# BaratiLab/GAMD

Measured on AMD Instinct MI355X. Metric: atom-steps/sec (force eval + integrate), 10k-atom LJ box, higher is better.
Workload: dtype f32; 1 GPU; C2: 10 000-atom LJ box, rho*=0.5, L=92.29 A, cutoff 3.0 sigma=10.2 A, fp32, 4 conv layers x 128, random-init weights (seed 0), 1 box per GPU; n_atoms=10000, boxes=1, launch=single process

## Files before the change

gamd_amd/_lib.py:

```python
from __future__ import annotations

import ctypes as C
import os

_HERE = os.path.dirname(os.path.abspath(__file__))
LIB_PATH = os.environ.get("GAMD_LIB") or os.path.join(_HERE, "libgamd_hip.so")


class GamdConfig(C.Structure):
    _fields_ = [("n_atoms", C.c_int32), ("kind", C.c_int32), ("n_layers", C.c_int32),
                ("use_bond", C.c_int32), ("nbr_flavour", C.c_int32), ("device", C.c_int32),
                ("cutoff", C.c_float), ("box", C.c_float * 3), ("edge_capacity", C.c_int64),
                ("keep_stages", C.c_int32), ("edge_dtype", C.c_int32),
                ("encoding_size", C.c_int32), ("edge_embedding_dim", C.c_int32), ("hidden_dim", C.c_int32),
                ("no_expand_edge", C.c_int32), ("neighbor_skin", C.c_float), ("self_loop_mode", C.c_int32),
                ("kernel_select", C.c_int32), ("small_tile_limit", C.c_int32), ("n_boxes", C.c_int32)]


_MD_EXT = [("mass_h_amu", C.c_float), ("length_per_nm", C.c_float), ("rigid_water", C.c_int32),
           ("r_oh", C.c_float), ("r_hh", C.c_float), ("remove_cm_motion", C.c_int32)]


class GamdNhcParams(C.Structure):
    _fields_ = [("dt_ps", C.c_float), ("mass_amu", C.c_float), ("temperature_k", C.c_float),
# ... 45 lines not shown
TRAJ_FIELDS = {"x": 1, "v": 2, "f": 4, "image": 8}
FORCE_SOURCE = {"network": 0, "classical": 1}


_vp, _i32, _i64 = C.c_void_p, C.c_int32, C.c_int64
SYMBOLS = {
    "gamd_version": (C.c_char_p, []),
    "gamd_last_error": (C.c_char_p, []),
    "gamd_create": (_i32, [C.POINTER(GamdConfig), C.POINTER(_vp)]),
    "gamd_destroy": (_i32, [_vp]),
    "gamd_load_weight": (_i32, [_vp, C.c_char_p, _vp, C.POINTER(_i64), _i32]),
    "gamd_finalize_weights": (_i32, [_vp]),
    "gamd_set_scaler": (_i32, [_vp, C.c_double, C.c_double]),
    "gamd_set_bonds": (_i32, [_vp, _vp, _i64]),
    "gamd_forces_async": (_i32, [_vp, _vp, _vp, C.POINTER(C.c_float), _vp, _vp, _vp]),
    "gamd_set_node_features": (_i32, [_vp, _vp]),
    "gamd_get_device_flags": (_i32, [_vp, C.POINTER(_i32)]),
    "gamd_sync_status": (_i32, [_vp, _vp]),
    "gamd_forces_host": (_i32, [_vp, _vp, _vp, C.POINTER(C.c_float), _vp, _i32, _vp]),
    "gamd_forces": (_i32, [_vp, _vp, _vp, C.POINTER(C.c_float), _vp, _vp, _vp]),
    "gamd_forces_edges": (_i32, [_vp, _vp, _vp, C.POINTER(C.c_float), _vp, _vp, _i64, _vp, _vp, _vp]),
    "gamd_build_neighbors": (_i32, [_vp, _vp, _vp, C.POINTER(C.c_float), _vp]),
    "gamd_get_counts": (_i32, [_vp, C.POINTER(_i64), C.POINTER(_i64), C.POINTER(_i64)]),
    "gamd_get_skin_stats": (_i32, [_vp, C.POINTER(_i64), C.POINTER(_i64), C.POINTER(_i64)]),
    "gamd_debug_get": (_i32, [_vp, _i32, _vp, C.c_size_t]),
    "gamd_md_run": (_i32, [_vp, _vp, _vp, _vp, _vp, C.POINTER(C.c_float), C.POINTER(GamdMdParams), _i64, _vp]),
    "gamd_md_run_nhc": (_i32, [_vp, _vp, _vp, _vp, _vp, C.POINTER(C.c_float), C.POINTER(GamdNhcParams), _vp, _i64, _vp]),
    "gamd_report_configure": (_i32, [_vp, C.POINTER(GamdReportParams)]),
    "gamd_report_reset": (_i32, [_vp]),
    "gamd_report_read": (_i32, [_vp, _vp, _vp, _vp, _vp, _i64, C.POINTER(_i64), _vp, _i64, C.POINTER(_i64), C.POINTER(_i64),
                                C.POINTER(_i32)]),
    "gamd_traj_configure": (_i32, [_vp, C.POINTER(GamdTrajParams)]),
    "gamd_traj_reset": (_i32, [_vp]),
    "gamd_traj_read_frames": (_i32, [_vp, _vp, _i64, _i64, _vp, _vp, _vp, _vp, _vp, C.POINTER(_i64), C.POINTER(_i64)]),
    "gamd_traj_read_dynamics": (_i32, [_vp, _vp, _vp, _vp, _i64, C.POINTER(_i64), C.POINTER(C.c_uint64), _vp, C.POINTER(_i32)]),
    "gamd_struct_configure": (_i32, [_vp, C.POINTER(GamdStructParams)]),
    "gamd_struct_reset": (_i32, [_vp]),
    "gamd_struct_read": (_i32, [_vp, _vp, _vp, _i64, _vp, _i64, _vp, _i64, C.POINTER(_i64), C.POINTER(_i32)]),
    "gamd_classical_configure": (_i32, [_vp, C.POINTER(GamdClassicalParams)]),
    "gamd_classical_reset": (_i32, [_vp]),
    "gamd_classical_read": (_i32, [_vp, _vp, _vp, _vp, _i64, C.POINTER(_i64), C.POINTER(_i64), _vp, _i64]),
    "gamd_classical_eval": (_i32, [_vp, _vp, C.POINTER(C.c_float), C.c_float, _vp, _vp, _vp, _vp, _vp]),
    "gamd_md_force_source": (_i32, [_vp, _i32]),
    "gamd_minimize": (_i32, [_vp, _vp, C.POINTER(C.c_float), C.c_float, _vp, _vp, C.POINTER(GamdMinimizeParams), _vp, _vp]),
    "gamd_water_configure": (_i32, [_vp, C.POINTER(GamdWaterParams)]),
    "gamd_water_reset": (_i32, [_vp]),
# ... 41 lines not shown
```

gamd_amd/csrc/conv_edge.hip:

```cpp
#include "gamd_common.h"
#include "gamd_internal.h"

#include <cstdlib>

namespace {

constexpr int conv_lds_floats(bool l0) { return 2 * GAMD_WFRAG_FLOATS + 3 * 128; }

template <bool F2, typename Post, typename Mid>
__device__ __forceinline__ void gemm128_post(const f32x4* W, int lane, const f32x16 (&X)[4], f32x16 (&acc)[4], Post post, Mid mid) {
#pragma unroll
    for (int tp = 0; tp < 4; ++tp) {
        if (tp == 1) mid();
#pragma unroll
        for (int t = 0; t < 4; ++t) {
#pragma unroll
            for (int q = 0; q < 4; ++q) {
                const f32x4 w = W[((tp * 4 + t) * 4 + q) * 64 + lane];
#pragma unroll
                for (int j = 0; j < 4; ++j) {
                    const float x = X[t][q * 4 + j];
                    acc[tp] = F2 ? mfma32(x, w[j], acc[tp]) : mfma32(w[j], x, acc[tp]);
                }
                if (tp > 0) post(tp - 1, t * 4 + q);
            }
        }
    }
#pragma unroll
    for (int g = 0; g < 16; ++g) post(3, g);
}

template <int N>
__device__ __forceinline__ void phase_barrier() {
    asm volatile("s_waitcnt vmcnt(%0) lgkmcnt(0)" ::"n"(N) : "memory");
    __builtin_amdgcn_s_barrier();
}

__device__ __forceinline__ void load_e_tile(const float* __restrict__ e_frag, int tile, int lane, f32x16 (&X)[4]) {
    const f32x4* ef = (const f32x4*)e_frag + (size_t)tile * 16 * 64;
#pragma unroll
    for (int t = 0; t < 4; ++t)
#pragma unroll
        for (int q = 0; q < 4; ++q) {
            const f32x4 v = gamd_load_stream(&ef[(t * 4 + q) * 64 + lane]);
#pragma unroll
            for (int j = 0; j < 4; ++j) X[t][q * 4 + j] = v[j];
        }
}

template <bool TIME, bool L0>
__global__ void __launch_bounds__(512, 2) k_conv_edge(ConvEdgeArgs a) {
    if (a.devflags[DEVFLAG_FROZEN]) return;
    extern __shared__ __attribute__((aligned(16))) float lds[];
    float* buf0 = lds + (L0 ? 3 * 128 : 0);
    float* buf1 = buf0 + GAMD_WFRAG_FLOATS;
    float* vb1 = L0 ? lds : buf1 + GAMD_WFRAG_FLOATS;
    float* vb3 = vb1 + 128;
    float* vb4 = vb3 + 128;
    float* vSD0 = vb4;

    const int tid = threadIdx.x, lane = tid & 63, slot = lane & 31, half = lane >> 5;
    const int wave = __builtin_amdgcn_readfirstlane(tid >> 6);
    const unsigned lane16 = (unsigned)lane * 16u;
    int E = a.counters[CNT_E];
    if ((long long)E > a.e_cap) E = (int)a.e_cap;
    const int n_tiles = (E + GAMD_TILE - 1) / GAMD_TILE;
    const int n_units = (n_tiles + 3) / 4;
    int first, end, step;
    gamd_xcd_range(n_units, blockIdx.x, gridDim.x, first, end, step);
    if (first >= end) return;
    const int n_iter = ((end - first + step - 1) / step + 1) / 2;
    const int wsub = wave & 3, whalf = wave >> 2;
    const bool early = whalf == 0;
    auto tile_of = [&](int it) {
        const int u = first + (2 * it + whalf) * step;
        return (it < n_iter && u < end) ? u * 4 + wsub : n_tiles;
    };
    auto stage = [&](const float* gw, float* buf) { gamd_stage_weight_raw_contig<8>(gw, buf, wave, lane16); };

    long long tacc[16];
#pragma unroll
    for (int i = 0; i < 16; ++i) tacc[i] = 0;
    long long tprev = 0;
#define TMARK(i) do { if (TIME) { const long long tn__ = (long long)__builtin_readcyclecounter(); tacc[i] += tn__ - tprev; tprev = tn__; } } while (0)

    if (tid < 128) {
        vb1[tid] = a.b1[tid]; vb3[tid] = a.b3[tid];
        if (L0) vSD0[tid] = a.S[tid] + a.D[tid];
        else vb4[tid] = a.b4[tid];
    }
    stage(a.w1p, buf0);

    f32x16 RA[4], RB[4], RC[4];
    auto init_b4 = [&]() {
// ... 105 lines not shown
            gemm128_post<false>((const f32x4*)by, lane, RB, RA,
                                [&](int tp, int g) { RA[tp][g] = gamd_silu_hw(RA[tp][g]); },
                                [&]() { FENCE(); stage(a.w3p, bx); FENCE(); });
            TMARK(4);
        } else {
            stage(a.w3p, bx);
        }
        phase_barrier<0>();
        asm volatile("" ::"v"(mask), "v"(p0), "v"(src_n));
        TMARK(5);
        if (active) {
            const unsigned bl = (unsigned)__ballot(src != a.zero_row) >> (4 * half);
            const unsigned real = (bl & 0xFu) | ((bl >> 4) & 0xF0u) | ((bl >> 8) & 0xF00u) | ((bl >> 12) & 0xF000u);
#pragma unroll
            for (int tp = 0; tp < 4; ++tp) {
                const float b = vb3[32 * tp + slot];
#pragma unroll
                for (int r = 0; r < 16; ++r) RC[tp][r] = ((real >> r) & 1u) ? b : GAMD_L0_PAD;
            }
            TMARK(7);
            const unsigned keep_bits = ~(mask << 1);
            gemm128_post<true>((const f32x4*)bx, lane, RA, RC, [&](int tp, int r) {
                RC[tp][r] = gamd_l0_acc(RC[tp][r], (r > 0 && ((keep_bits >> r) & 1u)) ? RC[tp][r - 1] : 0.f);
            }, [&]() { FENCE(); if (it + 1 < n_iter) stage(a.w1p, by); FENCE(); });
            pend_ends = mask;
            if (nvalid > 0 && !((mask >> (nvalid - 1)) & 1u)) pend_ends |= 1u << (nvalid - 1);
            pend_p = p0;
            TMARK(10);
        } else {
            if (it + 1 < n_iter) stage(a.w1p, by);
        }
        if (!early) phase_barrier<0>();
        TMARK(11);
        if (active_n) load_e_tile(a.e_frag, tile_n, lane, RA);
        TMARK(12);
        if (early) early_barrier(active_n);
        TMARK(13);
        tile = tile_n; active = active_n; src = src_n;
    }
    } else {
    for (int it = 0; it < n_iter; ++it) {
        const int x0 = tile * GAMD_TILE + 16 * half;
        int nvalid = E - x0;
        nvalid = !active ? 0 : (nvalid >= 16 ? 16 : (nvalid <= 0 ? 0 : nvalid));
        const int tile_n = tile_of(it + 1);
        const bool active_n = tile_n < n_tiles;
        int src_n = a.zero_row, dst_n = src_n;

        if (active) {
            load_bias_chain(vb1, half, RB);
            TMARK(0);
            gemm128_post<false>((const f32x4*)buf0, lane, RA, RB,
                                [&](int tp, int g) { RB[tp][g] = gamd_silu_hw(RB[tp][g]); },
// ... 35 lines not shown
        }
        if (active_n) {
            const int xn = tile_n * GAMD_TILE + gamd_pi(slot);
            if (xn < E) { src_n = GAMD_CHK_RANGE(a.sticky, a.col[xn], 0, a.zero_row, GAMD_CHK_CONV_SRC); dst_n = GAMD_CHK_RANGE(a.sticky, a.erow[xn], 0, a.zero_row, GAMD_CHK_CONV_DST); }
        }
        if (active) {
            load_bias_chain(vb3, half, RB);
            TMARK(7);
            gemm128_post<false>((const f32x4*)buf0, lane, RC, RB,
                                [&](int tp, int g) { RB[tp][g] = gamd_silu_hw(RB[tp][g]); },
                                [&]() { FENCE(); stage(a.w4p, buf1); FENCE(); });
            TMARK(8);
        } else {
            stage(a.w4p, buf1);
        }
        phase_barrier<0>();
        asm volatile("" ::"v"(mask), "v"(p0), "v"(src_n), "v"(dst_n));
        TMARK(9);
        if (active) {
            init_b4();
            const unsigned keep_bits = ~(mask << 1);
            gemm128_post<true>((const f32x4*)buf1, lane, RB, RC, [&](int tp, int r) {
                RC[tp][r] = gamd_msg_acc(RA[r >> 2][(r & 3) * 4 + tp], RC[tp][r], (r > 0 && ((keep_bits >> r) & 1u)) ? RC[tp][r - 1] : 0.f);
            }, [&]() { FENCE(); if (it + 1 < n_iter) stage(a.w1p, buf0); FENCE(); });
            pend_ends = mask;
            if (nvalid > 0 && !((mask >> (nvalid - 1)) & 1u)) pend_ends |= 1u << (nvalid - 1);
            pend_p = p0;
            TMARK(10);
        } else {
            if (it + 1 < n_iter) stage(a.w1p, buf0);
        }
        if (!early) phase_barrier<0>();
        TMARK(11);
        if (active_n) load_e_tile(a.e_frag, tile_n, lane, RA);
        TMARK(12);
        if (early) early_barrier(active_n);
        TMARK(13);
        tile = tile_n; active = active_n; src = src_n; dst = dst_n;
    }
    }
#undef FENCE
    piece_stores();
    if (TIME && a.tdbg && lane == 0) {
#pragma unroll
        for (int i = 0; i < 16; ++i) a.tdbg[((size_t)blockIdx.x * 8 + wave) * 16 + i] = tacc[i];
    }
#undef TMARK
}

template <bool TIME, bool L0>
int launch(const ConvEdgeArgs& a, int n_blocks, hipStream_t st) {
    const size_t lds = sizeof(float) * conv_lds_floats(L0);
    static PerDeviceOnce once;
    if (int e = gamd_allow_dynamic_lds(once, (int)lds, k_conv_edge<TIME, L0>)) return e;
    hipLaunchKernelGGL((k_conv_edge<TIME, L0>), dim3(n_blocks), dim3(512), lds, st, a);
    GAMD_CHECK_LAUNCH();
    return 0;
}

}

int launch_conv_edge(const ConvEdgeArgs& a, int n_blocks, hipStream_t st) {
#ifdef GAMD_PROFILING
    static const bool timed = getenv("GAMD_CONV_TIME") != nullptr;
    if (timed) return launch<true, false>(a, n_blocks, st);
// ... 12 lines not shown
```

gamd_amd/csrc/gamd_api.hip:

```cpp
#include "gamd_host.h"

#include <algorithm>
#include <cmath>
#include <cstddef>
#include <cstdlib>
#include <cstring>
#include <deque>

static_assert(sizeof(gamd_config) == 96 && offsetof(gamd_config, n_boxes) == 88 && offsetof(gamd_config, edge_capacity) == 40,
              "gamd_config layout is part of the C ABI (gamd_amd/_lib.py mirrors it)");

namespace {

bool small_path(const gamd_handle* h) { return h->use_small; }

int fill_com(gamd_handle* h, int enabled, MdCom* c) {
    c->enabled = enabled ? 1 : 0;
    c->blocks = std::max(1, std::min(16, (h->n_per_box + 1023) / 1024));
    c->partial = nullptr;
    if (!c->enabled) return 0;
    if (h->com_partial.ensure(sizeof(double) * 4 * (size_t)c->blocks * (size_t)h->n_boxes, true)) return fail(-12, "allocation failed");
    c->partial = h->com_partial.as<double>();
    return 0;
}
// ... 434 lines not shown
        ConvEdgeArgs ca{};
        ca.counters = h->cur_counters;
        ca.devflags = h->devflags.as<int>();
        ca.col = h->col.as<int>(); ca.erow = h->erow.as<int>();
        ca.chunk_piece = h->chunk_piece.as<int>(); ca.chunk_mask = h->chunk_mask.as<unsigned>();
        ca.e_frag = (h->update_edge && l > 0) ? h->e_frag2.as<float>() : h->e_frag.as<float>();
        ca.emb_out = (h->update_edge && l + 1 < h->L) ? h->e_emb.as<float>() : nullptr;
        ca.hn = h->hn.as<float>(); ca.S = h->S.as<float>(); ca.D = h->D.as<float>();
        if (l0 && l == 0) { ca.hn = h->l0_hn.as<float>(); ca.S = h->l0_S.as<float>(); ca.D = h->l0_D.as<float>(); }
        const LayerDev& ld = h->layers[l];
        ca.w1p = ld.w1p; ca.w2p = ld.w2p; ca.w3p = ld.w3p; ca.w4p = ld.w4p; ca.w16p = ld.w16p;
        ca.b1 = ld.b1; ca.b3 = ld.b3; ca.b4 = ld.b4;
        const bool hoist = l == 0 && h->l0_hoist;
        if (hoist) { ca.w3p = ld.w3p_l0; ca.b3 = ld.b3_l0; }
        ca.partial = h->partial.as<float>();
        ca.piece_cap = h->piece_cap;
        ca.sticky = h->sticky_dev;
        ca.e_cap = h->e_cap;
        ca.zero_row = h->n;
#ifdef GAMD_CHECKED
        { static const bool inject = getenv("GAMD_CHK_INJECT") != nullptr; if (inject) ca.zero_row = 0; }
#endif
        ca.tdbg = h->tdbg.as<long long>();
        if ((r = tev_begin(l))) return r;
        r = h->DT > 1 ? launch_conv_edge_wide_d(ca, h->EHT, h->HT, h->DT, h->n_cu, st)
            : h->wide_conv ? (h->cfg.edge_dtype == GAMD_EDGE_F16X3 ? launch_conv_edge_f16x3_wide(ca, h->EHT, h->HT, h->n_cu, st)
                            : h->cfg.edge_dtype == GAMD_EDGE_BF16 ? launch_conv_edge_bf16_wide(ca, h->EHT, h->HT, h->n_cu, st)
                            : (half_quantum && ca.w16p && !ca.emb_out) ? launch_conv_edge_wide16(ca, h->EHT, h->HT, h->n_cu, st)
                            : small_tiles > 0 ? launch_conv_edge_small_wide(ca, h->EHT, h->HT, small_tiles, st)
                                              : launch_conv_edge_wide(ca, h->EHT, h->HT, h->n_cu, st))
            : h->cfg.edge_dtype == GAMD_EDGE_BF16 ? launch_conv_edge_bf16(ca, h->n_cu, st)
            : h->cfg.edge_dtype == GAMD_EDGE_F16X3 ? launch_conv_edge_f16x3(ca, h->n_cu, st)
            : hoist ? (small_tiles > 0 ? launch_conv_edge_small_l0(ca, small_tiles, st) : launch_conv_edge_l0(ca, h->n_cu, st))
            : small_tiles > 0 ? launch_conv_edge_small(ca, small_tiles, st) : launch_conv_edge(ca, h->n_cu, st);
        if (r) return fail(-1, "conv edge launch failed (%d)", r);
        if ((r = tev_end())) return r;
        mark("conv_edge");
        if (ca.emb_out) {
            EdgeUpdateArgs ua{};
            ua.counters = h->cur_counters; ua.devflags = h->devflags.as<int>(); ua.e_cap = h->e_cap;
            ua.emb = ca.emb_out; ua.ln_g = ld.e_ln_g; ua.ln_b = ld.e_ln_b;
            ua.ln_inv_width = 1.0f / (float)h->Eh_true;
            ua.ln_n_pad = (float)(h->Eh - h->Eh_true);
            ua.e_frag_out = h->e_frag2.as<float>();
            if ((r = launch_edge_update(ua, h->HT, small_tiles > 0 ? std::max(1, small_tiles / 4) : 2 * h->n_cu, st)))
                return fail(-1, "edge update launch failed (%d)", r);
// ... 152 lines not shown
#ifdef GAMD_CHECKED
const char* gamd_version(void) { return "gamd_hip 0.1 (gfx950) checked"; }
#else
const char* gamd_version(void) { return "gamd_hip 0.1 (gfx950)"; }
#endif
const char* gamd_last_error(void) { return g_err; }

int32_t gamd_create(const gamd_config* cfg, gamd_handle** out) {
    if (!cfg || !out) return fail(-22, "null argument");
    if (cfg->n_atoms <= 0) return fail(-22, "n_atoms must be positive");
    if (cfg->n_boxes < 0 || cfg->n_boxes > (1 << 20)) return fail(-22, "n_boxes out of range");
    const int n_boxes = cfg->n_boxes > 1 ? cfg->n_boxes : 1;
    if ((long long)cfg->n_atoms * n_boxes >= (1 << 23) - 1)
        return fail(-22, "n_atoms x n_boxes = %lld: at most %d atoms per handle", (long long)cfg->n_atoms * n_boxes, (1 << 23) - 2);
    if (cfg->n_layers <= 0 || cfg->n_layers > 16) return fail(-22, "n_layers out of range");
    if (!(cfg->cutoff > 0.f)) return fail(-22, "cutoff must be positive");
    if (cfg->edge_dtype != GAMD_EDGE_F32 && cfg->edge_dtype != GAMD_EDGE_BF16 && cfg->edge_dtype != GAMD_EDGE_F16X3)
        return fail(-22, "unknown edge_dtype");
    if (!(cfg->neighbor_skin >= 0.f)) return fail(-22, "neighbor_skin must be >= 0");
    if (cfg->self_loop_mode != GAMD_SELF_LOOP_DGL07_NOOP && cfg->self_loop_mode != GAMD_SELF_LOOP_APPEND_ZERO_FEATURE)
        return fail(-22, "unknown self_loop_mode %d", cfg->self_loop_mode);
    if (cfg->self_loop_mode != GAMD_SELF_LOOP_DGL07_NOOP && cfg->edge_dtype != GAMD_EDGE_F32)
        return fail(-22, "self_loop_mode 1 is built for the fp32 edge dtype only");
    if (cfg->kernel_select & ~(GAMD_KSEL_FORCE_GENERIC_WIDTH | GAMD_KSEL_FORCE_HALF_QUANTUM | GAMD_KSEL_NO_LAYER0_HOIST))
        return fail(-22, "unknown kernel_select bits 0x%x", cfg->kernel_select);
    int ndev = 0;
    if (hipGetDeviceCount(&ndev) != hipSuccess || ndev <= 0)
        return fail(-19, "no HIP device available: libgamd_hip has no CPU fallback");
    if (cfg->device < 0 || cfg->device >= ndev) return fail(-22, "device %d out of range (%d visible)", cfg->device, ndev);
    DeviceGuard guard(cfg->device);
    hipDeviceProp_t prop;
    HIP_TRY(hipGetDeviceProperties(&prop, cfg->device));
    const int H_true = cfg->encoding_size ? cfg->encoding_size : 128, Eh_true = cfg->edge_embedding_dim ? cfg->edge_embedding_dim : 128;
    const int D_true = cfg->hidden_dim ? cfg->hidden_dim : 128;
    if (H_true < 1 || H_true > 256 || Eh_true < 1 || Eh_true > 256)
        return fail(-22, "encoding_size and edge_embedding_dim must be in [1, 256] (got %d, %d)", H_true, Eh_true);
    if (D_true < 1 || D_true > 256) return fail(-22, "hidden_dim must be in [1, 256] (got %d)", D_true);
    const int Dp = D_true <= 128 ? 128 : 256;
    if (Dp > 128 && cfg->edge_dtype != GAMD_EDGE_F32)
        return fail(-22, "hidden_dim above 128 is built for edge_dtype f32 only (got hidden_dim %d)", D_true);
    const int H = H_true <= 128 ? 128 : 256, Eh = Eh_true <= 128 ? 128 : 256;
    const bool exact128 = H_true == 128 && Eh_true == 128 && D_true == 128;
    const bool generic = H != 128 || Eh != 128 || cfg->no_expand_edge;
    if (cfg->edge_dtype != GAMD_EDGE_F32 && H == 256 && (long long)cfg->n_atoms * n_boxes > (1ll << 22) - 2)
        return fail(-22, "bf16 / split-fp16 with encoding_size > 128: at most 2^22 - 2 atoms per handle (32-bit byte offsets into hn)");
    gamd_handle* h = new gamd_handle();
    h->obs = observers_new();
// ... 681 lines not shown
    if ((r = enqueue_forward(h, pos_dev, species_dev, out_norm_dev, out_denorm_dev, (hipStream_t)stream, nullptr, nullptr,
                             nullptr, &el)))
        return r;
    HIP_TRY(hipStreamSynchronize((hipStream_t)stream));
    h->sticky_host[STICKY_EDGE_OVERFLOW] = 0;
    if (h->counters_host[CNT_OVERFLOW]) {
        const int why = h->counters_host[CNT_OVERFLOW];
        h->counters_host[CNT_OVERFLOW] = 0;
        if ((r = clear_devflags(h))) return r;
        if (why == 2) return fail(-22, "edge list references an atom index outside [0, n_atoms)");
        return fail(-34, "edge buffers overflowed unexpectedly");
    }
    return status;
}

int32_t gamd_get_counts(gamd_handle* h, int64_t* n_edges, int64_t* n_pieces, int64_t* edge_capacity) {
    if (!h) return fail(-22, "null handle");
    if (n_edges) *n_edges = h->counters_host[CNT_E];
    if (n_pieces) *n_pieces = h->counters_host[CNT_PIECES];
    if (edge_capacity) *edge_capacity = h->e_cap;
    return 0;
}

int32_t gamd_get_skin_stats(gamd_handle* h, int64_t* n_rebuilds, int64_t* n_candidates, int64_t* candidate_capacity) {
    if (!h) return fail(-22, "null handle");
    if (n_rebuilds) *n_rebuilds = h->sticky_host[STICKY_REBUILDS];
    if (n_candidates) *n_candidates = h->sticky_host[STICKY_NCAND];
    if (candidate_capacity) *candidate_capacity = h->cand_cap;
    return 0;
}

int32_t gamd_debug_get(gamd_handle* h, int32_t what, void* host_out, size_t bytes) {
    if (!h || !host_out) return fail(-22, "null argument");
    DeviceGuard guard(h->dev);
    InitStream init(h->init_stream);
    HIP_TRY(hipDeviceSynchronize());
    const size_t n = (size_t)h->n;
    const size_t E = (size_t)std::min<long long>(h->counters_host[CNT_E], h->e_cap);
    const void* src = nullptr;
    size_t avail = 0;
    if (what == GAMD_DBG_PERM) { src = h->perm.p; avail = sizeof(int) * n; }
    else if (what == GAMD_DBG_ROWPTR) { src = h->row_ptr.p; avail = sizeof(int) * (n + 1); }
    else if (what == GAMD_DBG_COL) { src = h->col.p; avail = sizeof(int) * E; }
    else if (what == GAMD_DBG_EFRAG) { src = h->e_frag.p; avail = sizeof(float) * 4096 * (size_t)h->EHT * ((E + 31) / 32); }
    else if (what == GAMD_DBG_FEAT) {
        if (!h->cfg.keep_stages) return fail(-22, "FEAT needs keep_stages=1");
// ... 205 lines not shown
```

gamd_amd/csrc/gamd_host.h:

```cpp
#pragma once
#include "../../include/gamd_hip.h"
#include "gamd_common.h"
#include "gamd_internal.h"

#include <cstdarg>
#include <cstdio>
#include <map>
#include <string>
#include <vector>

#pragma GCC visibility push(hidden)

inline thread_local char g_err[512] = "";

inline int fail(int code, const char* fmt, ...) {
    va_list ap;
    va_start(ap, fmt);
    vsnprintf(g_err, sizeof(g_err), fmt, ap);
    va_end(ap);
    return code;
}

#define HIP_TRY(expr)                                                                              \
    do {                                                                                           \
// ... 80 lines not shown
bool observers_sampled(const gamd_handle* h, long long s);
int observers_enqueue(gamd_handle* h, long long s);
int drive_check_source(gamd_handle* h);
int drive_check_run(gamd_handle* h, const float* box, const uint8_t* species_dev);
int drive_enqueue(gamd_handle* h);

struct gamd_handle {
    gamd_config cfg{};
    int dev = 0;
    int n = 0, L = 0, n_feat = 44, n_cu = 256;
    int n_boxes = 1, n_per_box = 0;
    bool use_small = false;
    DevBuf boxes_dev, box_shift;
    std::vector<float> boxes_host;
    int H = 128, Eh = 128, HT = 1, EHT = 1;
    int H_true = 128, Eh_true = 128, D_true = 128;
    int Dp = 128, DT = 1;
    int norm_bn = 0;
    bool update_edge = false;
    bool node_f16 = false;
    bool wide_enc = false, wide_conv = false;
    bool l0_hoist = false;
    long long small_tile_limit = 512;
    std::map<std::string, HostTensor> host_w;
    bool finalized = false;
    double scaler_mean = 0.0, scaler_var = 1.0;

    DevBuf wblob;
    std::vector<LayerDev> layers;
    const float *enc_w1p = nullptr, *enc_w2p = nullptr, *enc_w3p = nullptr, *enc_b1 = nullptr, *enc_b2 = nullptr,
                *enc_b3 = nullptr, *enc_lng = nullptr, *enc_lnb = nullptr, *centers = nullptr;
    const float *node_emb = nullptr, *nenc_w = nullptr, *nenc_b = nullptr;
    const float *dec_w1p = nullptr, *dec_b1 = nullptr, *dec_w2 = nullptr, *dec_b2 = nullptr;
    float length_mean = 0.f, length_std = 1.f;
    RbfGrid rbf{};

    DevBuf pos_w, pos_s, cell_of, perm, inv_perm, deg, row_ptr, na_excl, bond_nbr;
    DevBuf hbuf, hn, S, D, P, f_norm, f_den;
    DevBuf l0_h, l0_hn, l0_S, l0_D, l0_P;
    DevBuf cell_cnt, cell_fill, cell_start;
    int ncell_cap = 0;
    long long e_cap = 0;
    long long piece_cap = 0;
    DevBuf col, erow, chunk_piece, chunk_mask, e_frag, partial, feat_dbg, e_emb, e_frag2;
    DevBuf counters, tdbg, tmp_eid, ke_partial, com_partial;
    DevBuf cnt2;
// ... 56 lines not shown
```

gamd_amd/csrc/gamd_internal.h:

```cpp
#pragma once
#include <hip/hip_runtime.h>
#include <stdint.h>
#include <atomic>
#include "gamd_common.h"

enum { CNT_E = 0, CNT_PIECES = 1, CNT_OVERFLOW = 2, CNT_TILES = 3, CNT_REBUILD = 4, CNT_NCAND = 5,
       CNT_CAND_MAX = 6,
       CNT_COUNT = 8 };
enum { STICKY_EDGE_OVERFLOW = 0, STICKY_CAND_OVERFLOW = 1, STICKY_REBUILDS = 2, STICKY_NCAND = 3,
       STICKY_NONFINITE = 4,
       STICKY_CHECK_CODE = 5, STICKY_CHECK_VALUE = 6, STICKY_CHECK_LINE = 7,
       STICKY_COUNT = 8 };
enum { GAMD_CHK_CELL = 101, GAMD_CHK_CAND = 102, GAMD_CHK_EDGE_POS = 103, GAMD_CHK_PERM = 104, GAMD_CHK_ENC_SRC = 111, GAMD_CHK_ENC_DST = 112,
       GAMD_CHK_CONV_SRC = 121, GAMD_CHK_CONV_DST = 122, GAMD_CHK_PIECE = 123, GAMD_CHK_NODE_PIECES = 131, GAMD_CHK_INJECTED = 199 };
#ifdef GAMD_CHECKED
template <typename T>
__device__ __forceinline__ T gamd_chk_range(int* sticky, T v, long long lo, long long hi, int code, int line) {
    if ((long long)v >= lo && (long long)v <= hi) return v;
    if (sticky && sticky[STICKY_CHECK_CODE] == 0) {
        sticky[STICKY_CHECK_VALUE] = (int)v;
        sticky[STICKY_CHECK_LINE] = line;
        __threadfence_system();
        sticky[STICKY_CHECK_CODE] = code;
    }
// ... 171 lines not shown
int launch_edge_encode_wide_d(const EncArgs& a, int eht, int dt, int n_blocks, hipStream_t st);

struct ConvEdgeArgs {
    const int* counters;
    const int* devflags;
    const int* col;
    const int* erow;
    const int* chunk_piece;
    const unsigned* chunk_mask;
    const float* e_frag;
    const float* hn;
    const float* S;
    const float* D;
    const float* w1p; const float* w2p; const float* w3p; const float* w4p;
    const float* w16p;
    const float* b1; const float* b3; const float* b4;
    float* partial;
    long long e_cap;
    int zero_row;
    long long* tdbg;
    int* sticky;
    long long piece_cap;
    float* emb_out;
};
int launch_conv_edge(const ConvEdgeArgs& a, int n_blocks, hipStream_t st);
int launch_conv_edge_l0(const ConvEdgeArgs& a, int n_blocks, hipStream_t st);
int launch_conv_edge_bf16(const ConvEdgeArgs& a, int n_blocks, hipStream_t st);
int launch_conv_edge_small(const ConvEdgeArgs& a, int n_blocks, hipStream_t st);
int launch_conv_edge_small_l0(const ConvEdgeArgs& a, int n_blocks, hipStream_t st);
int launch_conv_edge_small_wide(const ConvEdgeArgs& a, int eht, int ht, int n_blocks, hipStream_t st);
int launch_conv_edge_f16x3(const ConvEdgeArgs& a, int n_blocks, hipStream_t st);
int launch_conv_edge_wide(const ConvEdgeArgs& a, int eht, int ht, int n_blocks, hipStream_t st);
int launch_conv_edge_wide16(const ConvEdgeArgs& a, int eht, int ht, int n_blocks, hipStream_t st);
int launch_conv_edge_wide_d(const ConvEdgeArgs& a, int eht, int ht, int dt, int n_blocks, hipStream_t st);
int launch_conv_edge_f16x3_wide(const ConvEdgeArgs& a, int eht, int ht, int n_blocks, hipStream_t st);
int launch_conv_edge_bf16_wide(const ConvEdgeArgs& a, int eht, int ht, int n_blocks, hipStream_t st);

struct EdgeUpdateArgs {
    const int* counters;
    const int* devflags;
    long long e_cap;
    const float* emb;
    const float* ln_g; const float* ln_b;
    float ln_inv_width, ln_n_pad;
    float* e_frag_out;
};
// ... 286 lines not shown
```

gamd_amd/engine.py:

```python
from __future__ import annotations

import ctypes as C
import os
from typing import Dict, Optional, Sequence, Tuple, Union

import numpy as np
import torch

from . import _lib
from ._lib import GamdClassicalParams, GamdMinimizeParams, GamdWaterParams, GamdReportParams, GamdStructParams, GamdTrajParams, GamdConfig, GamdMdParams, GamdNhcParams, TRAJ_FIELDS, check
from .weights import ModelConfig, infer_config, validate_state_dict

ArrayLike = Union[np.ndarray, torch.Tensor]

KIND = {"lj": 0, "water": 1, "dynbox": 1}
FLAVOUR = {"jaxmd": 0, "torch": 1}
SELF_LOOP = {"dgl07_noop": 0, "append_zero_feature_loops": 1}
KSEL_FORCE_GENERIC_WIDTH = 1
KSEL_NO_LAYER0_HOIST = 4


def _box3(box) -> np.ndarray:
    b = np.asarray(box, dtype=np.float64).reshape(-1)
    if b.size == 1:
        b = np.repeat(b, 3)
    if b.size != 3:
        raise ValueError("box must be a scalar or 3 values")
    return b.astype(np.float32)


def _boxes(box, n_boxes: int) -> np.ndarray:
    b = np.asarray(box, dtype=np.float64)
    if b.ndim == 0 or b.size == 1 or (b.ndim == 1 and b.size == 3):
        return np.tile(_box3(b), (n_boxes, 1))
    if b.ndim == 2 and b.shape == (n_boxes, 3):
        return b.astype(np.float32)
    if (b.ndim == 1 and b.size == n_boxes) or (b.ndim == 2 and b.shape == (n_boxes, 1)):
        return np.repeat(b.reshape(-1).astype(np.float32)[:, None], 3, axis=1)
    raise ValueError(f"box must be a scalar, 3 values, [{n_boxes}, 1] or [{n_boxes}, 3] ({n_boxes} boxes)")


def _rdf_from_counts(counts, frames: int, r_max: float, n_by_class, vol: float):
# ... 442 lines not shown
            raise ValueError("edge_idx must be [2, E]")
        st = self._lib.gamd_forces_edges(self._h, C.c_void_p(p.data_ptr()),
                                         C.c_void_p(s.data_ptr()) if s is not None else None, self._box_arg(box),
                                         C.c_void_p(e[0].data_ptr()), C.c_void_p(e[1].data_ptr()), int(e.shape[1]),
                                         C.c_void_p(self._out.data_ptr()), C.c_void_p(self._out_den.data_ptr()),
                                         self._stream())
        self.last_status = check(st, "gamd_forces_edges")
        out = self._out_den if denormalize else self._out
        return out if inplace else out.clone()

    def build_neighbors(self, pos: ArrayLike, box=None, species=None) -> int:
        p = self._dev_pos(pos)
        s = self._dev_species(species)
        st = self._lib.gamd_build_neighbors(self._h, C.c_void_p(p.data_ptr()),
                                            C.c_void_p(s.data_ptr()) if s is not None else None,
                                            self._box_arg(box), self._stream())
        return check(st, "gamd_build_neighbors")

    def counts(self) -> Tuple[int, int, int]:
        e, p, c = C.c_int64(), C.c_int64(), C.c_int64()
        check(self._lib.gamd_get_counts(self._h, C.byref(e), C.byref(p), C.byref(c)), "gamd_get_counts")
        return e.value, p.value, c.value

    def skin_stats(self) -> Tuple[int, int, int]:
        r, c, cap = C.c_int64(), C.c_int64(), C.c_int64()
        check(self._lib.gamd_get_skin_stats(self._h, C.byref(r), C.byref(c), C.byref(cap)), "gamd_get_skin_stats")
        return r.value, c.value, cap.value

    def _dbg(self, what: int, shape, dtype) -> np.ndarray:
        out = np.empty(shape, dtype=dtype)
        check(self._lib.gamd_debug_get(self._h, what, out.ctypes.data_as(C.c_void_p), out.nbytes), "gamd_debug_get")
        return out

    def debug_partial(self) -> np.ndarray:
        return self._dbg(6, (self.counts()[1], 128 * ((self.cfg.encoding_size + 127) // 128)), np.float32)

    def debug_perm(self) -> np.ndarray:
        return self._dbg(0, (self.n_total,), np.int32)

    def debug_csr(self) -> Tuple[np.ndarray, np.ndarray]:
        e = self.counts()[0]
        return self._dbg(1, (self.n_total + 1,), np.int32), self._dbg(2, (e,), np.int32)

    def debug_edges(self) -> np.ndarray:
        perm = self.debug_perm().astype(np.int64)
        row_ptr, col = self.debug_csr()
# ... 361 lines not shown
```

include/gamd_hip.h:

```cpp
#ifndef GAMD_HIP_H
#define GAMD_HIP_H

#include <stdint.h>
#include <stddef.h>

#ifdef __cplusplus
extern "C" {
#endif

typedef struct gamd_handle gamd_handle;

enum { GAMD_EDGE_F32 = 0, GAMD_EDGE_BF16 = 1, GAMD_EDGE_F16X3 = 2 };

enum { GAMD_KIND_LJ = 0, GAMD_KIND_WATER = 1 };
enum { GAMD_NBR_JAXMD = 0, GAMD_NBR_TORCH = 1 };

typedef struct gamd_config {
    int32_t n_atoms;
    int32_t kind;
    int32_t n_layers;
    int32_t use_bond;
    int32_t nbr_flavour;
    int32_t device;
    float cutoff;
    float box[3];
    int64_t edge_capacity;
    int32_t keep_stages;
    int32_t edge_dtype;
    int32_t encoding_size;
    int32_t edge_embedding_dim;
    int32_t hidden_dim;
    int32_t no_expand_edge;
    float neighbor_skin;
    int32_t self_loop_mode;
    int32_t kernel_select;
    int32_t small_tile_limit;
    int32_t n_boxes;
} gamd_config;
enum { GAMD_SELF_LOOP_DGL07_NOOP = 0, GAMD_SELF_LOOP_APPEND_ZERO_FEATURE = 1 };
enum { GAMD_KSEL_FORCE_GENERIC_WIDTH = 1, GAMD_KSEL_FORCE_HALF_QUANTUM = 2, GAMD_KSEL_NO_LAYER0_HOIST = 4 };

const char* gamd_version(void);
const char* gamd_last_error(void);

int32_t gamd_create(const gamd_config* cfg, gamd_handle** out);
int32_t gamd_destroy(gamd_handle* h);

int32_t gamd_load_weight(gamd_handle* h, const char* name, const float* data, const int64_t* shape, int32_t ndim);
int32_t gamd_finalize_weights(gamd_handle* h);

int32_t gamd_set_scaler(gamd_handle* h, double mean, double var);

int32_t gamd_set_bonds(gamd_handle* h, const int32_t* bonds, int64_t n_bonds);

int32_t gamd_forces_async(gamd_handle* h, const float* pos_dev, const uint8_t* species_dev, const float* box,
                          float* out_norm_dev, float* out_denorm_dev, void* stream);

int32_t gamd_set_node_features(gamd_handle* h, const float* feat_dev);

int32_t gamd_sync_status(gamd_handle* h, void* stream);

int32_t gamd_get_device_flags(gamd_handle* h, int32_t flags[4]);

int32_t gamd_forces(gamd_handle* h, const float* pos_dev, const uint8_t* species_dev, const float* box,
                    float* out_norm_dev, float* out_denorm_dev, void* stream);

int32_t gamd_forces_host(gamd_handle* h, const float* pos_host, const uint8_t* species_dev, const float* box, float* out_host,
                         int32_t denormalize, void* stream);

int32_t gamd_forces_edges(gamd_handle* h, const float* pos_dev, const uint8_t* species_dev, const float* box,
                          const int32_t* centre_dev, const int32_t* neigh_dev, int64_t n_edges,
                          float* out_norm_dev, float* out_denorm_dev, void* stream);

int32_t gamd_build_neighbors(gamd_handle* h, const float* pos_dev, const uint8_t* species_dev, const float* box,
                             void* stream);

int32_t gamd_get_counts(gamd_handle* h, int64_t* n_edges, int64_t* n_pieces, int64_t* edge_capacity);

int32_t gamd_get_skin_stats(gamd_handle* h, int64_t* n_rebuilds, int64_t* n_candidates, int64_t* candidate_capacity);

enum {
    GAMD_DBG_PERM = 0,
    GAMD_DBG_ROWPTR = 1,
    GAMD_DBG_COL = 2,
    GAMD_DBG_EFRAG = 3,
    GAMD_DBG_FEAT = 4,
    GAMD_DBG_CYCLES = 5,
    GAMD_DBG_PARTIAL = 6,
    GAMD_DBG_H0 = 16
};
int32_t gamd_debug_get(gamd_handle* h, int32_t what, void* host_out, size_t bytes);

typedef struct gamd_md_params {
    float dt_ps;
    float mass_amu;
    float temperature_k;
    float gamma_per_ps;
    uint64_t seed;
    uint64_t first_step;
    float mass_h_amu;
// ... 147 lines not shown
```

Baseline: 3.380 million atom-steps/s.

## Split conv-edge tail tiles across all workgroups to balance the last wave

The conv edge kernel now hands each workgroup whole 4-tile units only up to the largest multiple of 4×grid tiles. The few leftover tiles (at most two per workgroup) go through a new tail path in which four waves each compute a quarter of the 128-wide GEMMs, using an extra LDS exchange buffer. The goal is to remove load imbalance where a handful of workgroups process an extra unit while the rest sit idle. The cost is more LDS per block, which may lower occupancy, plus a more complex code path that can be disabled with a kernel_select bit.

```diff
diff --git a/gamd_amd/_lib.py b/gamd_amd/_lib.py
--- a/gamd_amd/_lib.py
+++ b/gamd_amd/_lib.py
@@ -91,6 +91,7 @@
     "gamd_forces_edges": (_i32, [_vp, _vp, _vp, C.POINTER(C.c_float), _vp, _vp, _i64, _vp, _vp, _vp]),
     "gamd_build_neighbors": (_i32, [_vp, _vp, _vp, C.POINTER(C.c_float), _vp]),
     "gamd_get_counts": (_i32, [_vp, C.POINTER(_i64), C.POINTER(_i64), C.POINTER(_i64)]),
+    "gamd_debug_conv_tail": (_i32, [_vp, C.POINTER(_i32), C.POINTER(_i32), C.POINTER(_i32)]),
     "gamd_get_skin_stats": (_i32, [_vp, C.POINTER(_i64), C.POINTER(_i64), C.POINTER(_i64)]),
     "gamd_debug_get": (_i32, [_vp, _i32, _vp, C.c_size_t]),
     "gamd_md_run": (_i32, [_vp, _vp, _vp, _vp, _vp, C.POINTER(C.c_float), C.POINTER(GamdMdParams), _i64, _vp]),
diff --git a/gamd_amd/csrc/conv_edge.hip b/gamd_amd/csrc/conv_edge.hip
--- a/gamd_amd/csrc/conv_edge.hip
+++ b/gamd_amd/csrc/conv_edge.hip
@@ -5,7 +5,7 @@
 
 namespace {
 
-constexpr int conv_lds_floats(bool l0) { return 2 * GAMD_WFRAG_FLOATS + 3 * 128; }
+constexpr int conv_lds_floats(bool l0) { return 2 * GAMD_WFRAG_FLOATS + 3 * 128 + GAMD_TILE * GAMD_XLD; }
 
 template <bool F2, typename Post, typename Mid>
 __device__ __forceinline__ void gemm128_post(const f32x4* W, int lane, const f32x16 (&X)[4], f32x16 (&acc)[4], Post post, Mid mid) {
@@ -28,6 +28,37 @@
     }
 #pragma unroll
     for (int g = 0; g < 16; ++g) post(3, g);
+}
+
+template <bool F2>
+__device__ __forceinline__ void gemm_quarter_lds(const f32x4* W, int lane, int quarter, bool hasB, const f32x16 (&XA)[4], f32x16& accA,
+                                                 const f32x16 (&XB)[4], f32x16& accB) {
+    const f32x4* Wq = W + quarter * 16 * 64 + lane;
+    f32x4 wc[4], wn[4];
+#pragma unroll
+    for (int q = 0; q < 4; ++q) wc[q] = Wq[q * 64];
+#pragma unroll
+    for (int t = 0; t < 4; ++t) {
+        if (t < 3) {
+#pragma unroll
+            for (int q = 0; q < 4; ++q) wn[q] = Wq[((t + 1) * 4 + q) * 64];
+        }
+#pragma unroll
+        for (int q = 0; q < 4; ++q)
+#pragma unroll
+            for (int j = 0; j < 4; ++j) accA = F2 ? mfma32(XA[t][q * 4 + j], wc[q][j], accA) : mfma32(wc[q][j], XA[t][q * 4 + j], accA);
+        if (hasB) {
+#pragma unroll
+            for (int q = 0; q < 4; ++q)
+#pragma unroll
+                for (int j = 0; j < 4; ++j) accB = F2 ? mfma32(XB[t][q * 4 + j], wc[q][j], accB) : mfma32(wc[q][j], XB[t][q * 4 + j], accB);
+        }
+        __builtin_amdgcn_sched_barrier(0);
+#pragma unroll
+        for (int q = 0; q < 4; ++q) wc[q] = wn[q];
+    }
+    asm volatile("s_nop 15\n\ts_nop 3" ::: "memory");
+    __builtin_amdgcn_sched_barrier(0);
 }
 
 template <int N>
@@ -66,10 +97,13 @@
     if ((long long)E > a.e_cap) E = (int)a.e_cap;
     const int n_tiles = (E + GAMD_TILE - 1) / GAMD_TILE;
     const int n_units = (n_tiles + 3) / 4;
+    const int tail0 = n_tiles / (4 * (int)gridDim.x) * (4 * (int)gridDim.x);
+    const bool split = a.tail_split && n_tiles > tail0 && n_tiles - tail0 <= 2 * (int)gridDim.x;
+    const bool has_tail = split && tail0 + (int)blockIdx.x < n_tiles;
     int first, end, step;
-    gamd_xcd_range(n_units, blockIdx.x, gridDim.x, first, end, step);
-    if (first >= end) return;
-    const int n_iter = ((end - first + step - 1) / step + 1) / 2;
+    gamd_xcd_range(split ? tail0 / 4 : n_units, blockIdx.x, gridDim.x, first, end, step);
+    if (first >= end && !has_tail) return;
+    const int n_iter = first < end ? ((end - first + step - 1) / step + 1) / 2 : 0;
     const int wsub = wave & 3, whalf = wave >> 2;
     const bool early = whalf == 0;
     auto tile_of = [&](int it) {
@@ -221,13 +255,13 @@
             const unsigned keep_bits = ~(mask << 1);
             gemm128_post<true>((const f32x4*)bx, lane, RA, RC, [&](int tp, int r) {
                 RC[tp][r] = gamd_l0_acc(RC[tp][r], (r > 0 && ((keep_bits >> r) & 1u)) ? RC[tp][r - 1] : 0.f);
-            }, [&]() { FENCE(); if (it + 1 < n_iter) stage(a.w1p, by); FENCE(); });
+            }, [&]() { FENCE(); if (it + 1 < n_iter || has_tail) stage(a.w1p, by); FENCE(); });
             pend_ends = mask;
             if (nvalid > 0 && !((mask >> (nvalid - 1)) & 1u)) pend_ends |= 1u << (nvalid - 1);
             pend_p = p0;
             TMARK(10);
         } else {
-            if (it + 1 < n_iter) stage(a.w1p, by);
+            if (it + 1 < n_iter || has_tail) stage(a.w1p, by);
         }
         if (!early) phase_barrier<0>();
         TMARK(11);
@@ -309,13 +343,13 @@
             const unsigned keep_bits = ~(mask << 1);
             gemm128_post<true>((const f32x4*)buf1, lane, RB, RC, [&](int tp, int r) {
                 RC[tp][r] = gamd_msg_acc(RA[r >> 2][(r & 3) * 4 + tp], RC[tp][r], (r > 0 && ((keep_bits >> r) & 1u)) ? RC[tp][r - 1] : 0.f);
-            }, [&]() { FENCE(); if (it + 1 < n_iter) stage(a.w1p, buf0); FENCE(); });
+            }, [&]() { FENCE(); if (it + 1 < n_iter || has_tail) stage(a.w1p, buf0); FENCE(); });
             pend_ends = mask;
             if (nvalid > 0 && !((mask >> (nvalid - 1)) & 1u)) pend_ends |= 1u << (nvalid - 1);
             pend_p = p0;
             TMARK(10);
         } else {
-            if (it + 1 < n_iter) stage(a.w1p, buf0);
+            if (it + 1 < n_iter || has_tail) stage(a.w1p, buf0);
         }
         if (!early) phase_barrier<0>();
         TMARK(11);
@@ -328,6 +362,171 @@
     }
 #undef FENCE
     piece_stores();
+
+    if (has_tail) {
+        float* const xbuf = lds + 2 * GAMD_WFRAG_FLOATS + 3 * 128;
+        const int flip = (L0 && (n_iter & 1)) ? GAMD_WFRAG_FLOATS : 0;
+        float* const s1 = buf0 + flip;
+        float* const s2 = buf0 + (GAMD_WFRAG_FLOATS - flip);
+        const int tA = tail0 + (int)blockIdx.x, tB = tA + (int)gridDim.x;
+        const bool hasB = tB < n_tiles;
+        const bool cw = wave < 4;
+        const int quarter = wsub;
+        f32x16 XA[4], XB[4], accA, accB, gA, gB;
+        int srcA = a.zero_row, srcB = a.zero_row;
+
+        auto tile_in = [&](int t, int& s, f32x16 (&X)[4], f32x16& dq) {
+            const int x = t * GAMD_TILE + gamd_pi(slot);
+            int d = a.zero_row;
+            if (x < E) {
+                s = GAMD_CHK_RANGE(a.sticky, a.col[x], 0, a.zero_row, GAMD_CHK_CONV_SRC);
+                if (!L0) d = GAMD_CHK_RANGE(a.sticky, a.erow[x], 0, a.zero_row, GAMD_CHK_CONV_DST);
+            }
+            load_e_tile(a.e_frag, t, lane, X);
+            if (!L0) dq = load_slice(a.D + (size_t)d * GAMD_H, quarter, half);
+        };
+        auto silu16 = [](f32x16& v) {
+#pragma unroll
+            for (int r = 0; r < 16; ++r) v[r] = gamd_silu_hw(v[r]);
+        };
+        auto xchg = [&](const f32x16& mine, f32x16 (&X)[4]) {
+            if (cw) exchange(xbuf, quarter, slot, half, mine, X);
+            else { __syncthreads(); __syncthreads(); }
+        };
+        auto tile_pieces = [&](int t, unsigned& mask, int& p0) {
+            mask = a.chunk_mask[t * 2 + half];
+            p0 = GAMD_CHK_RANGE(a.sticky, a.chunk_piece[t * 2 + half], 0, a.piece_cap - 17, GAMD_CHK_PIECE);
+        };
+        auto tile_stores = [&](int t, const f32x16& acc, unsigned mask, int p) {
+            int nvalid = E - (t * GAMD_TILE + 16 * half);
+            nvalid = nvalid >= 16 ? 16 : (nvalid <= 0 ? 0 : nvalid);
+            unsigned ends = mask;
+            if (nvalid > 0 && !((mask >> (nvalid - 1)) & 1u)) ends |= 1u << (nvalid - 1);
+            while (__any(ends != 0)) {
+                if (ends != 0) {
+                    const int r = __builtin_ctz(ends);
+                    ends &= ends - 1;
+                    float v = acc[0];
+#pragma unroll
+                    for (int k = 1; k < 16; ++k) v = (r == k) ? acc[k] : v;
+                    a.partial[(size_t)p * GAMD_H + 4 * slot + quarter] = v;
+                    ++p;
+                }
+            }
+        };
+
+        if (cw) {
+            tile_in(tA, srcA, XA, gA);
+            if (hasB) tile_in(tB, srcB, XB, gB);
+        }
+        __builtin_amdgcn_s_waitcnt(0x0F70);
+        stage(a.w2p, s2);
+        if (cw) {
+            accA = load_slice(vb1, quarter, half);
+            accB = accA;
+            gemm_quarter_lds<false>((const f32x4*)s1, lane, quarter, hasB, XA, accA, XB, accB);
+            silu16(accA);
+            if (hasB) silu16(accB);
+        }
+        xchg(accA, XA);
+        if (hasB) xchg(accB, XB);
+        phase_barrier<0>();
+
+        if (cw) {
+            if (L0) { accA = load_slice(vSD0, quarter, half); accB = accA; }
+            else {
+                accA = gA; accB = gB;
+                gA = load_slice(a.S + (size_t)srcA * GAMD_H, quarter, half);
+                if (hasB) gB = load_slice(a.S + (size_t)srcB * GAMD_H, quarter, half);
+            }
+        }
+        stage(a.w3p, s1);
+        if (cw) {
+            gemm_quarter_lds<false>((const f32x4*)s2, lane, quarter, hasB, XA, accA, XB, accB);
+            if (!L0) accA += gA;
+            silu16(accA);
+            if (hasB) {
+                if (!L0) accB += gB;
+                silu16(accB);
+            }
+        }
+        xchg(accA, XA);
+        if (hasB) xchg(accB, XB);
+        phase_barrier<0>();
+
+        unsigned maskA = 0, maskB = 0;
+        int pA = 0, pB = 0;
+        if constexpr (L0) {
+            if (cw) {
+                tile_pieces(tA, maskA, pA);
+                if (hasB) tile_pieces(tB, maskB, pB);
+                const float b = vb3[32 * quarter + slot];
+                auto l0_start = [&](int src, f32x16& acc) {
+                    const unsigned bl = (unsigned)__ballot(src != a.zero_row) >> (4 * half);
+                    const unsigned real = (bl & 0xFu) | ((bl >> 4) & 0xF0u) | ((bl >> 8) & 0xF00u) | ((bl >> 12) & 0xF000u);
+#pragma unroll
+                    for (int r = 0; r < 16; ++r) acc[r] = ((real >> r) & 1u) ? b : GAMD_L0_PAD;
+                };
+                auto l0_sum = [&](unsigned mask, f32x16& acc) {
+                    const unsigned keep_bits = ~(mask << 1);
+#pragma unroll
+                    for (int r = 0; r < 16; ++r) acc[r] = gamd_l0_acc(acc[r], (r > 0 && ((keep_bits >> r) & 1u)) ? acc[r - 1] : 0.f);
+                };
+                l0_start(srcA, accA);
+                l0_start(srcB, accB);
+                gemm_quarter_lds<true>((const f32x4*)s1, lane, quarter, hasB, XA, accA, XB, accB);
+                l0_sum(maskA, accA);
+                tile_stores(tA, accA, maskA, pA);
+                if (hasB) {
+                    l0_sum(maskB, accB);
+                    tile_stores(tB, accB, maskB, pB);
+                }
+            }
+        } else {
+            if (cw) {
+                auto hn_in = [&](int src, f32x16& hq) {
+                    const unsigned soff = (unsigned)src << 9, mine = 16u * (unsigned)slot + 4u * (unsigned)quarter;
+#pragma unroll
+                    for (int r = 0; r < 16; ++r) {
+                        const unsigned o = (unsigned)__shfl((int)soff, (r & 3) + 8 * (r >> 2) + 4 * half, 64);
+                        hq[r] = *(const float*)((const char*)a.hn + (o + mine));
+                    }
+                };
+                tile_pieces(tA, maskA, pA);
+                hn_in(srcA, gA);
+                if (hasB) { tile_pieces(tB, maskB, pB); hn_in(srcB, gB); }
+            }
+            stage(a.w4p, s2);
+            if (cw) {
+                accA = load_slice(vb3, quarter, half);
+                accB = accA;
+                gemm_quarter_lds<false>((const f32x4*)s1, lane, quarter, hasB, XA, accA, XB, accB);
+                silu16(accA);
+                if (hasB) silu16(accB);
+            }
+            xchg(accA, XA);
+            if (hasB) xchg(accB, XB);
+            phase_barrier<0>();
+            if (cw) {
+                const float b = vb4[32 * quarter + slot];
+#pragma unroll
+                for (int r = 0; r < 16; ++r) accA[r] = b;
+                accB = accA;
+                gemm_quarter_lds<true>((const f32x4*)s2, lane, quarter, hasB, XA, accA, XB, accB);
+                auto msg_tile = [&](unsigned mask, const f32x16& hq, f32x16& acc) {
+                    const unsigned keep_bits = ~(mask << 1);
+#pragma unroll
+                    for (int r = 0; r < 16; ++r) acc[r] = gamd_msg_acc(hq[r], acc[r], (r > 0 && ((keep_bits >> r) & 1u)) ? acc[r - 1] : 0.f);
+                };
+                msg_tile(maskA, gA, accA);
+                tile_stores(tA, accA, maskA, pA);
+                if (hasB) {
+                    msg_tile(maskB, gB, accB);
+                    tile_stores(tB, accB, maskB, pB);
+                }
+            }
+        }
+    }
     if (TIME && a.tdbg && lane == 0) {
 #pragma unroll
         for (int i = 0; i < 16; ++i) a.tdbg[((size_t)blockIdx.x * 8 + wave) * 16 + i] = tacc[i];
diff --git a/gamd_amd/csrc/gamd_api.hip b/gamd_amd/csrc/gamd_api.hip
--- a/gamd_amd/csrc/gamd_api.hip
+++ b/gamd_amd/csrc/gamd_api.hip
@@ -480,6 +480,8 @@
         { static const bool inject = getenv("GAMD_CHK_INJECT") != nullptr; if (inject) ca.zero_row = 0; }
 #endif
         ca.tdbg = h->tdbg.as<long long>();
+        ca.tail_split = (h->cfg.kernel_select & GAMD_KSEL_NO_TAIL_SPLIT) ? 0 : 1;
+        h->last_conv_blocks = (h->DT > 1 || h->wide_conv || h->cfg.edge_dtype != GAMD_EDGE_F32 || small_tiles > 0) ? 0 : h->n_cu;
         if ((r = tev_begin(l))) return r;
         r = h->DT > 1 ? launch_conv_edge_wide_d(ca, h->EHT, h->HT, h->DT, h->n_cu, st)
             : h->wide_conv ? (h->cfg.edge_dtype == GAMD_EDGE_F16X3 ? launch_conv_edge_f16x3_wide(ca, h->EHT, h->HT, h->n_cu, st)
@@ -678,7 +680,7 @@
         return fail(-22, "unknown self_loop_mode %d", cfg->self_loop_mode);
     if (cfg->self_loop_mode != GAMD_SELF_LOOP_DGL07_NOOP && cfg->edge_dtype != GAMD_EDGE_F32)
         return fail(-22, "self_loop_mode 1 is built for the fp32 edge dtype only");
-    if (cfg->kernel_select & ~(GAMD_KSEL_FORCE_GENERIC_WIDTH | GAMD_KSEL_FORCE_HALF_QUANTUM | GAMD_KSEL_NO_LAYER0_HOIST))
+    if (cfg->kernel_select & ~(GAMD_KSEL_FORCE_GENERIC_WIDTH | GAMD_KSEL_FORCE_HALF_QUANTUM | GAMD_KSEL_NO_LAYER0_HOIST | GAMD_KSEL_NO_TAIL_SPLIT))
         return fail(-22, "unknown kernel_select bits 0x%x", cfg->kernel_select);
     int ndev = 0;
     if (hipGetDeviceCount(&ndev) != hipSuccess || ndev <= 0)
@@ -1406,6 +1408,17 @@
     return 0;
 }
 
+int32_t gamd_debug_conv_tail(gamd_handle* h, int32_t* n_workgroups, int32_t* whole_units, int32_t* leftover_tiles) {
+    if (!h) return fail(-22, "null handle");
+    const long long e = std::min<long long>(h->counters_host[CNT_E], h->e_cap);
+    const int g = h->last_conv_blocks, t = (int)((e + GAMD_TILE - 1) / GAMD_TILE);
+    const int u = g > 0 ? t / (4 * g) : 0;
+    if (n_workgroups) *n_workgroups = g;
+    if (whole_units) *whole_units = u;
+    if (leftover_tiles) *leftover_tiles = g > 0 ? t - 4 * g * u : 0;
+    return 0;
+}
+
 int32_t gamd_get_skin_stats(gamd_handle* h, int64_t* n_rebuilds, int64_t* n_candidates, int64_t* candidate_capacity) {
     if (!h) return fail(-22, "null handle");
     if (n_rebuilds) *n_rebuilds = h->sticky_host[STICKY_REBUILDS];
diff --git a/gamd_amd/csrc/gamd_host.h b/gamd_amd/csrc/gamd_host.h
--- a/gamd_amd/csrc/gamd_host.h
+++ b/gamd_amd/csrc/gamd_host.h
@@ -126,6 +126,7 @@
     bool wide_enc = false, wide_conv = false;
     bool l0_hoist = false;
     long long small_tile_limit = 512;
+    int last_conv_blocks = 0;
     std::map<std::string, HostTensor> host_w;
     bool finalized = false;
     double scaler_mean = 0.0, scaler_var = 1.0;
diff --git a/gamd_amd/csrc/gamd_internal.h b/gamd_amd/csrc/gamd_internal.h
--- a/gamd_amd/csrc/gamd_internal.h
+++ b/gamd_amd/csrc/gamd_internal.h
@@ -217,6 +217,7 @@
     int* sticky;
     long long piece_cap;
     float* emb_out;
+    int tail_split;
 };
 int launch_conv_edge(const ConvEdgeArgs& a, int n_blocks, hipStream_t st);
 int launch_conv_edge_l0(const ConvEdgeArgs& a, int n_blocks, hipStream_t st);
diff --git a/gamd_amd/engine.py b/gamd_amd/engine.py
--- a/gamd_amd/engine.py
+++ b/gamd_amd/engine.py
@@ -18,6 +18,7 @@
 SELF_LOOP = {"dgl07_noop": 0, "append_zero_feature_loops": 1}
 KSEL_FORCE_GENERIC_WIDTH = 1
 KSEL_NO_LAYER0_HOIST = 4
+KSEL_NO_TAIL_SPLIT = 8
 
 
 def _box3(box) -> np.ndarray:
@@ -506,6 +507,11 @@
         check(self._lib.gamd_get_counts(self._h, C.byref(e), C.byref(p), C.byref(c)), "gamd_get_counts")
         return e.value, p.value, c.value
 
+    def debug_conv_tail(self) -> Tuple[int, int, int]:
+        g, u, r = C.c_int32(), C.c_int32(), C.c_int32()
+        check(self._lib.gamd_debug_conv_tail(self._h, C.byref(g), C.byref(u), C.byref(r)), "gamd_debug_conv_tail")
+        return g.value, u.value, r.value
+
     def skin_stats(self) -> Tuple[int, int, int]:
         r, c, cap = C.c_int64(), C.c_int64(), C.c_int64()
         check(self._lib.gamd_get_skin_stats(self._h, C.byref(r), C.byref(c), C.byref(cap)), "gamd_get_skin_stats")
diff --git a/include/gamd_hip.h b/include/gamd_hip.h
--- a/include/gamd_hip.h
+++ b/include/gamd_hip.h
@@ -38,7 +38,7 @@
     int32_t n_boxes;
 } gamd_config;
 enum { GAMD_SELF_LOOP_DGL07_NOOP = 0, GAMD_SELF_LOOP_APPEND_ZERO_FEATURE = 1 };
-enum { GAMD_KSEL_FORCE_GENERIC_WIDTH = 1, GAMD_KSEL_FORCE_HALF_QUANTUM = 2, GAMD_KSEL_NO_LAYER0_HOIST = 4 };
+enum { GAMD_KSEL_FORCE_GENERIC_WIDTH = 1, GAMD_KSEL_FORCE_HALF_QUANTUM = 2, GAMD_KSEL_NO_LAYER0_HOIST = 4, GAMD_KSEL_NO_TAIL_SPLIT = 8 };
 
 const char* gamd_version(void);
 const char* gamd_last_error(void);
@@ -76,6 +76,8 @@
                              void* stream);
 
 int32_t gamd_get_counts(gamd_handle* h, int64_t* n_edges, int64_t* n_pieces, int64_t* edge_capacity);
+
+int32_t gamd_debug_conv_tail(gamd_handle* h, int32_t* n_workgroups, int32_t* whole_units, int32_t* leftover_tiles);
 
 int32_t gamd_get_skin_stats(gamd_handle* h, int64_t* n_rebuilds, int64_t* n_candidates, int64_t* candidate_capacity);
 
```

Result: no change. 3.397 million atom-steps/s, median of 6 (+0.5%).
